# Vandermode/ELD

Hardware: AMD Instinct MI355X
Metric: raw megapixels/sec (noise-synth + U-Net step) (higher is better)
Workload: dtype f32; 1 GPU; BASELINE.json configs[1]: full ELD noise model (PGRU, SonyA7S2 params) on 4x1424x2128 packed raw + U-Net fp32 train step (fwd, L1, bwd, Adam), 8 frames per GPU; images_per_gpu=8, global_batch=8, parallelism=dp1

## Files before the change

### eld_amd/csrc/conv.h

```cpp
#pragma once
#include "common.h"

typedef float f32x16 __attribute__((ext_vector_type(16)));
typedef float f32x2 __attribute__((ext_vector_type(2)));
typedef __bf16 bf16x2_hw __attribute__((ext_vector_type(2)));

enum ConvMode { CONV_3X3 = 0, CONV_1X1 = 1, CONV_GATHER2X2 = 2 };
enum ConvEpi { EPI_FWD = 0, EPI_CONVT_FWD = 1, EPI_GRAD = 2 };

typedef unsigned short bf16_t;
enum ConvDtype { DT_F32 = 0, DT_BF16 = 1 };

struct ConvArgs {
    const void* in0;
    const void* in1;
    int C0, C1;
    const void* wp;
    int N, H, W;
    int Nout;
    int epi;
    const float* bias;
    int lrelu;
    void* out0;
    void* out1;
// ... 229 lines not shown
int launch_conv_x3w(const ConvArgs& a, hipStream_t st);
int bfd_slab_bn(int Nout, int K, int N, int H, int W);
__host__ __device__ inline size_t bfd_slab_bytes(int BN) { return (size_t)3 * BN * 64; }
int launch_conv_bfd(const ConvArgs& a, hipStream_t st);
int debug_kernel_mask(int set);
bool bfs_takes(int Nout, int K, int N, int H, int W);
int launch_conv_bfs(const ConvArgs& a, hipStream_t st);
bool bfw_takes(const ConvArgs& a);
int launch_conv_bfw(const ConvArgs& a, hipStream_t st);
int bfg_slab_bn(bool gather, int Nout, int Cs, int Cout_t, int N, int H, int W);
__host__ __device__ inline size_t bfg_slab_bytes(int BN) { return (size_t)BN * 64; }
int launch_conv_bfg(const ConvArgs& a, int mode, hipStream_t st);

#ifdef __HIPCC__
__device__ __forceinline__ int xcd_block(int on) {
    const int b = (int)blockIdx.x;
    if (!on) return b;
    const int n = (int)gridDim.x, q = n >> 3, r = n & 7, x = b & 7;
    return (x < r ? x * (q + 1) : r * (q + 1) + (x - r) * q) + (b >> 3);
}
#endif
__host__ __device__ inline void band_tile(int id, int tiles_x, int tiles_y, int BH, int& ty, int& tx) {
    if (BH <= 1) { ty = id / tiles_x; tx = id - ty * tiles_x; return; }
    const int full = tiles_x * BH, band = id / full, off = id - band * full;
    int bh = tiles_y - band * BH;
    if (bh > BH) bh = BH;
    tx = off / bh;
    ty = band * BH + (off - tx * bh);
}
int eld_tile_band();
enum { XCD_GEMM = 1, XCD_WGRAD8 = 2, XCD_WGRAD = 4, XCD_X3D = 8, XCD_X3W = 16, XCD_BF16 = 32, XCD_IGEMM = 64 };
int eld_xcd_mask();

struct WgradArgs {
    const void* g;
    int CA;
    const void* x0;
    const void* x1;
    int C0, C1;
    int N, H, W;
    float* part;
    float* bpart;
    float* xbpart;
    int CBp;
    int psplit;
    int tiles_x, tiles_y;
    int vp;
    int dtype;
    int algo;
    int wgrad8;
    int xcd;
    int band;
    const float* amax_g; const float* amax_x0; const float* amax_x1;
};

int launch_wgrad(const WgradArgs& a, int mode, hipStream_t st);
bool wgrad8_shape(int CA, int CBp, int& COB, int& JB, int& TH, int& TWo, bool bf16 = false);
int wgrad8_ntiles(int CA, int CBp, int N, int H, int W, bool bf16);
bool wgradt8_takes(int CA, int CB);
int wgradt8_ntiles(int N, int H, int W);
int launch_wgrad_reduce(const float* part, const float* bpart, float* wgrad, float* bgrad, int psplit, int T, int CA,
                        int CBp, int CBr, hipStream_t st, int bias_n = 0);
```

### eld_amd/csrc/conv_wgrad.hip

```cpp
#include <stdlib.h>
#include "conv.h"

#define TW 32
#define JB 32

typedef __bf16 bf16x8 __attribute__((ext_vector_type(8)));
typedef short s16x4 __attribute__((ext_vector_type(4)));
typedef int i32x4_t __attribute__((ext_vector_type(4)));
typedef _Float16 half8 __attribute__((ext_vector_type(8)));

enum { ALG_F32 = 0, ALG_BFM = 1, ALG_X3 = 2, ALG_H2 = 3 };

template <typename T, int MODE, int WCO, int TH, int ALG>
__global__ __launch_bounds__(256, 2) void wgrad_kernel(const WgradArgs a) {
    constexpr bool BFM = ALG == ALG_BFM, X3 = ALG == ALG_X3, H2 = ALG == ALG_H2;
    static_assert(!(X3 || H2) || sizeof(T) == 4, "x3 / h2: fp32 inputs");
    constexpr int ES = sizeof(T);
    constexpr int EPU = 16 / ES;
    constexpr int LES = X3 ? 6 : (BFM ? 2 : 4);
    constexpr int TAPS = MODE == CONV_3X3 ? 9 : 4;
    constexpr int WPIX = 4 / WCO;
    constexpr int COB = 32 * WCO;
    constexpr int TPIX = TH * TW;
    constexpr int PW = TPIX / WPIX;
// ... 320 lines not shown

    const int tid = threadIdx.x, lane = tid & 63, wave = tid >> 6;
    const int m = lane & 31, hi = lane >> 5;
    const int wco = wave % WCO, wci = (wave / WCO) % WCI, wpix = wave / (WCO * WCI);
    const int IB = a.CA / COB, JBn = a.CBp / JBK;
    int bid = xcd_block(a.xcd);
    const int jb = bid % JBn; bid /= JBn;
    const int ib = bid % IB;
    const int ps = bid / IB;
    const int i0 = ib * COB, j0 = jb * JBK;
    const bool do_bias = a.bpart != nullptr && jb == 0;

    f32x16 acc[TAPS];
#pragma unroll
    for (int t = 0; t < TAPS; ++t)
#pragma unroll
        for (int i = 0; i < 16; ++i) acc[t][i] = 0.f;
    float4 bsum4 = make_float4(0.f, 0.f, 0.f, 0.f), bsum4b = make_float4(0.f, 0.f, 0.f, 0.f);

    const int ntiles = a.tiles_x * a.tiles_y;
    const int VP = a.vp;
    const bool seam = VP % TH != 0;
    constexpr unsigned OOB = 0xFFFFFFF0u;
    constexpr int G_STEP = THREADS / G_Q;
    const int g_part = tid % G_Q, g_lp0 = tid / G_Q;
    const int g_px0 = g_lp0 % TWT, g_py0 = g_lp0 / TWT;
    const unsigned g_off0 = (unsigned)(g_px0 * a.CA + i0 + g_part * EPU) * (unsigned)ES;
    const int g_lds0 = ((g_part * EPU) >> 5) * GBLK + g_lp0 * 32 + ((g_part * EPU) & 31);
    auto g_pxy = [&](int it, int& dpx, int& dpy) {
        if (G_STEP >= TWT) { dpx = 0; dpy = it * (G_STEP / TWT); }
        else { dpx = (it * G_STEP) % TWT; dpy = (it * G_STEP) / TWT; }
    };
    const int x_part = (int)((unsigned)tid % (unsigned)XQ);
    int x_hyx[X_IT];
#pragma unroll
    for (int it = 0; it < X_IT; ++it) {
        const int hp = (int)((unsigned)(tid + it * THREADS) / (unsigned)XQ);
        const int hy = hp / (TWT + 2);
        x_hyx[it] = (hy << 8) | (hp - hy * (TWT + 2));
    }
    auto x_alive = [&](int it) { return (it + 1) * THREADS <= X_UNITS1 || (int)((unsigned)(tid + it * THREADS) / (unsigned)XQ) < X_PIX; };
    const char* xs[WCI]; int xC[WCI], xc0[WCI];
#pragma unroll
    for (int cb = 0; cb < WCI; ++cb) {
        const int c = j0 + cb * 32;
        if (c < a.C0) { xs[cb] = static_cast<const char*>(a.x0); xC[cb] = a.C0; xc0[cb] = c; }
        else if (c < a.C0 + a.C1) { xs[cb] = static_cast<const char*>(a.x1); xC[cb] = a.C1; xc0[cb] = c - a.C0; }
        else { xs[cb] = nullptr; xC[cb] = 32; xc0[cb] = 0; }
    }
    float4 rg[G_IT], rx[WCI][X_IT];
    const size_t g_img = (size_t)a.H * a.W * a.CA * ES;
    const unsigned g_rowc = (unsigned)(g_py0 * a.W * a.CA) * (unsigned)ES;
    auto load_tile = [&](int tile) {
        int ty, tx;
        band_tile(tile, a.tiles_x, a.tiles_y, a.band, ty, tx);
        const int v0 = ty * TH, x0 = tx * TWT;
        const int img0 = v0 / VP, vrel = v0 - img0 * VP;
        const int wrem = a.W - x0;
        if (!seam || VP - vrel > TH) {
            const __amdgpu_buffer_rsrc_t rs_g = __builtin_amdgcn_make_buffer_rsrc((void*)(static_cast<const char*>(a.g) + (size_t)img0 * g_img), 0, (int)g_img, 0x00020000);
            const int gbase = (vrel * a.W + x0) * a.CA * ES;
#pragma unroll
            for (int it = 0; it < G_IT; ++it) {
                int dpx, dpy;
                g_pxy(it, dpx, dpy);
                const unsigned off = g_off0 + g_rowc + (unsigned)((dpy * a.W + dpx) * a.CA) * (unsigned)ES;
                rg[it] = __builtin_bit_cast(float4, __builtin_amdgcn_raw_buffer_load_b128(rs_g, g_px0 + dpx < wrem ? (int)off : (int)OOB, gbase, 0));
            }
#pragma unroll
            for (int cb = 0; cb < WCI; ++cb) {
                const size_t x_img = (size_t)a.H * a.W * xC[cb] * ES;
                const __amdgpu_buffer_rsrc_t rs_x = __builtin_amdgcn_make_buffer_rsrc((void*)(xs[cb] ? xs[cb] + (size_t)img0 * x_img : nullptr), 0, xs[cb] ? (int)x_img : 0, 0x00020000);
#pragma unroll
                for (int it = 0; it < X_IT; ++it) {
                    const int gy = vrel - 1 + (x_hyx[it] >> 8), gx = x0 - 1 + (x_hyx[it] & 255);
                    const bool ok = x_alive(it) && (unsigned)gy < (unsigned)a.H && (unsigned)gx < (unsigned)a.W;
                    const unsigned off = ok ? (unsigned)((gy * a.W + gx) * xC[cb] + xc0[cb] + x_part * EPU) * (unsigned)ES : OOB;
                    rx[cb][it] = __builtin_bit_cast(float4, __builtin_amdgcn_raw_buffer_load_b128(rs_x, (int)off, 0, 0));
                }
            }
            return;
        }
        const int nimg = a.N - img0 < 2 ? a.N - img0 : 2;
        const int lim0 = a.H - vrel, nxt = VP - vrel;
        const __amdgpu_buffer_rsrc_t rs_g = __builtin_amdgcn_make_buffer_rsrc((void*)(static_cast<const char*>(a.g) + (size_t)img0 * g_img), 0, (int)(g_img * nimg), 0x00020000);
        const unsigned gb0 = (unsigned)((vrel * a.W + x0) * a.CA) * (unsigned)ES;
        const unsigned gb1 = (unsigned)(((a.H - nxt) * a.W + x0) * a.CA) * (unsigned)ES;
#pragma unroll
        for (int it = 0; it < G_IT; ++it) {
            int dpx, dpy;
            g_pxy(it, dpx, dpy);
            const int r = g_py0 + dpy;
            const bool second = r >= nxt;
            const bool ok = (r < lim0 || (second && r - nxt < a.H)) && g_px0 + dpx < wrem;
            const unsigned off = (second ? gb1 : gb0) + g_off0 + g_rowc + (unsigned)((dpy * a.W + dpx) * a.CA) * (unsigned)ES;
            rg[it] = __builtin_bit_cast(float4, __builtin_amdgcn_raw_buffer_load_b128(rs_g, ok ? (int)off : (int)OOB, 0, 0));
        }
#pragma unroll
        for (int cb = 0; cb < WCI; ++cb) {
            const size_t x_img = (size_t)a.H * a.W * xC[cb] * ES;
            const __amdgpu_buffer_rsrc_t rs_x = __builtin_amdgcn_make_buffer_rsrc((void*)(xs[cb] ? xs[cb] + (size_t)img0 * x_img : nullptr), 0, xs[cb] ? (int)(x_img * nimg) : 0, 0x00020000);
#pragma unroll
            for (int it = 0; it < X_IT; ++it) {
                const int r = (x_hyx[it] >> 8) - 1, gx = x0 - 1 + (x_hyx[it] & 255);
                const bool second = r >= nxt;
                const int wrow = second ? a.H + r - nxt : vrel + r;
                const bool rok = second ? r - nxt < a.H : (unsigned)(vrel + r) < (unsigned)a.H;
                const bool ok = x_alive(it) && rok && (unsigned)gx < (unsigned)a.W;
                const unsigned off = ok ? (unsigned)((wrow * a.W + gx) * xC[cb] + xc0[cb] + x_part * EPU) * (unsigned)ES : OOB;
                rx[cb][it] = __builtin_bit_cast(float4, __builtin_amdgcn_raw_buffer_load_b128(rs_x, (int)off, 0, 0));
            }
        }
    };
    auto put3 = [&](bf16_t* d, int plane_elems, const float4& raw) {
        if constexpr (ES == 2) { *reinterpret_cast<float4*>(d) = raw; return; }
        const unsigned x0 = __float_as_uint(raw.x), x1 = __float_as_uint(raw.y), x2 = __float_as_uint(raw.z), x3 = __float_as_uint(raw.w);
        const float r0 = raw.x - __uint_as_float(x0 & 0xFFFF0000u), r1 = raw.y - __uint_as_float(x1 & 0xFFFF0000u);
        const float r2 = raw.z - __uint_as_float(x2 & 0xFFFF0000u), r3 = raw.w - __uint_as_float(x3 & 0xFFFF0000u);
        const unsigned y0 = __float_as_uint(r0), y1 = __float_as_uint(r1), y2 = __float_as_uint(r2), y3 = __float_as_uint(r3);
        const unsigned z0 = __float_as_uint(r0 - __uint_as_float(y0 & 0xFFFF0000u)), z1 = __float_as_uint(r1 - __uint_as_float(y1 & 0xFFFF0000u));
        const unsigned z2 = __float_as_uint(r2 - __uint_as_float(y2 & 0xFFFF0000u)), z3 = __float_as_uint(r3 - __uint_as_float(y3 & 0xFFFF0000u));
        auto hp = [](unsigned lo, unsigned hi_) { return __builtin_amdgcn_perm(hi_, lo, 0x07060302u); };
        *reinterpret_cast<uint2*>(d) = make_uint2(hp(x0, x1), hp(x2, x3));
        *reinterpret_cast<uint2*>(d + plane_elems) = make_uint2(hp(y0, y1), hp(y2, y3));
        *reinterpret_cast<uint2*>(d + 2 * plane_elems) = make_uint2(hp(z0, z1), hp(z2, z3));
    };
    auto store_tile = [&]() {
#pragma unroll
        for (int it = 0; it < G_IT; ++it) {
            put3(ldsG + g_lds0 + it * G_STEP * 32, GPL, rg[it]);
            if (do_bias) {
                if constexpr (ES == 4) { bsum4.x += rg[it].x; bsum4.y += rg[it].y; bsum4.z += rg[it].z; bsum4.w += rg[it].w; }
                else {
                    const uint4 q = __builtin_bit_cast(uint4, rg[it]);
                    const float4 lo = unpack_bf4(make_uint2(q.x, q.y)), hi4 = unpack_bf4(make_uint2(q.z, q.w));
                    bsum4.x += lo.x; bsum4.y += lo.y; bsum4.z += lo.z; bsum4.w += lo.w;
                    bsum4b.x += hi4.x; bsum4b.y += hi4.y; bsum4b.z += hi4.z; bsum4b.w += hi4.w;
                }
            }
        }
#pragma unroll
        for (int cb = 0; cb < WCI; ++cb)
#pragma unroll
            for (int it = 0; it < X_IT; ++it)
                if (x_alive(it)) put3(ldsX + (cb * X_PIX + (int)((unsigned)(tid + it * THREADS) / (unsigned)XQ)) * 32 + x_part * EPU, XPL, rx[cb][it]);
    };

    const int gi = lane & 15, gg = lane >> 4;
    constexpr bool ROWSHARE = STREAM == 2;
    static_assert(!ROWSHARE || (NPC == 3 && TWT == 8 && WPIX == 1 && TH % 2 == 0), "row-shared fragments: fp32, 8-pixel-wide tiles, one pixel slice");
    constexpr int HS = TH / 2;
    const int lq0 = ROWSHARE ? HS * TWT * hi + (gi >> 2) : wpix * PW + 8 * hi + (gi >> 2);
    const int pyq = lq0 / TWT, pxq = lq0 - pyq * TWT;
    const bf16_t* gq = ldsG + wco * GBLK + lq0 * 32 + (gg & 1) * 16 + (gi & 3) * 4;
    const bf16_t* xq = ldsX + (wci * X_PIX + pyq * (TWT + 2) + pxq) * 32 + (gg & 1) * 16 + (gi & 3) * 4;
    auto tr8 = [](const bf16_t* p0) {
        const s16x4 lo = __builtin_amdgcn_ds_read_tr16_b64_v4i16((__attribute__((address_space(3))) s16x4*)p0);
        const s16x4 hi4 = __builtin_amdgcn_ds_read_tr16_b64_v4i16((__attribute__((address_space(3))) s16x4*)(p0 + 4 * 32));
        return __builtin_bit_cast(bf16x8, __builtin_shufflevector(lo, hi4, 0, 1, 2, 3, 4, 5, 6, 7));
    };

    if (ps < ntiles) load_tile(ps);
    for (int tile = ps; tile < ntiles; tile += a.psplit) {
        __syncthreads();
        store_tile();
        __syncthreads();
        if (tile + a.psplit < ntiles) load_tile(tile + a.psplit);
        if constexpr (ROWSHARE) {
            constexpr int GI[6] = {0, 1, 2, 0, 1, 0};
            constexpr int XI[6] = {2, 1, 0, 1, 0, 0};
            constexpr int NU = (HS + 2) * 3;
            bf16x8 gr[3][3], xf[2][3];
            auto readG = [&](int s_, bf16x8 (&g3)[3]) {
#pragma unroll
                for (int pc = 0; pc < 3; ++pc) g3[pc] = tr8(gq + pc * GPL + s_ * TWT * 32);
            };
            auto readF = [&](int a_, int kx, bf16x8 (&x3)[3]) {
#pragma unroll
                for (int pc = 0; pc < 3; ++pc) x3[pc] = tr8(xq + pc * XPL + (a_ * (TWT + 2) + kx) * 32);
            };
            readG(0, gr[0]);
            readF(0, 0, xf[0]);
#pragma unroll
            for (int u = 0; u < NU; ++u) {
                const int a_ = u / 3, kx = u % 3;
                if (u + 1 < NU) readF((u + 1) / 3, (u + 1) % 3, xf[(u + 1) & 1]);
                __builtin_amdgcn_sched_barrier(0);
#pragma unroll
                for (int ky = 2; ky >= 0; --ky) {
                    const int s_ = a_ - ky;
                    if (s_ >= 0 && s_ < HS) {
#pragma unroll
                        for (int q = 0; q < 6; ++q)
                            acc[3 * ky + kx] = __builtin_amdgcn_mfma_f32_32x32x16_bf16(gr[s_ % 3][GI[q]], xf[u & 1][XI[q]], acc[3 * ky + kx], 0, 0, 0);
                    }
                    if (ky == 2 && kx == 2 && a_ + 1 < HS) {
                        __builtin_amdgcn_sched_barrier(0);
                        readG(a_ + 1, gr[(a_ + 1) % 3]);
                    }
                }
                __builtin_amdgcn_sched_barrier(0);
            }
        } else
        if constexpr (NPC == 3 && STREAM == 1) {
            constexpr int GI[6] = {0, 1, 2, 0, 1, 0};
            constexpr int XI[6] = {2, 1, 0, 1, 0, 0};
            constexpr int NBLK = KSB * TAPS;
            bf16x8 ga[2][3], xb[2][3];
            auto readG = [&](int ks, bf16x8 (&g3)[3]) {
#pragma unroll
                for (int pc = 0; pc < 3; ++pc) g3[pc] = tr8(gq + pc * GPL + ks * 16 * 32);
            };
            auto readX = [&](int ks, int t, bf16x8 (&x3)[3]) {
                const int lrel = ks * 16, dy0 = lrel / TWT, dxp = lrel - dy0 * TWT;
                const int xoff = (dy0 + t / 3) * (TWT + 2) + dxp + t % 3;
#pragma unroll
                for (int pc = 0; pc < 3; ++pc) x3[pc] = tr8(xq + pc * XPL + xoff * 32);
            };
            readG(0, ga[0]);
            readX(0, 0, xb[0]);
// ... 25 lines not shown
                for (int tt = 0; tt < 3; ++tt) {
                    const int xoff = (dy0 + t0 / 3) * (TWT + 2) + dxp + tt;
#pragma unroll
                    for (int pc = 0; pc < NPC; ++pc) xb[tt][pc] = tr8(xq + pc * XPL + xoff * 32);
                }
                if constexpr (NPC == 3) {
                    constexpr int GI[6] = {0, 1, 2, 0, 1, 0};
                    constexpr int XI[6] = {2, 1, 0, 1, 0, 0};
#pragma unroll
                    for (int q = 0; q < 6; ++q)
#pragma unroll
                        for (int tt = 0; tt < 3; ++tt)
                            acc[t0 + tt] = __builtin_amdgcn_mfma_f32_32x32x16_bf16(ga[GI[q]], xb[tt][XI[q]], acc[t0 + tt], 0, 0, 0);
                } else {
#pragma unroll
                    for (int tt = 0; tt < 3; ++tt) acc[t0 + tt] = __builtin_amdgcn_mfma_f32_32x32x16_bf16(ga[0], xb[tt][0], acc[t0 + tt], 0, 0, 0);
                }
                __builtin_amdgcn_sched_barrier(0);
            }
        }
    }

    __syncthreads();
    float* red = lds;
    const size_t pbase = (size_t)ps * TAPS * a.CA * a.CBp;
    const int wt = wci * WCO + wco;
#pragma unroll
    for (int t = 0; t < TAPS; ++t) {
        if (WPIX > 1) {
            if (wpix > 0) {
#pragma unroll
                for (int i = 0; i < 16; ++i) red[(((wpix - 1) * (WCO * WCI) + wt) * 16 + i) * 64 + lane] = acc[t][i];
            }
            __syncthreads();
            if (wpix == 0) {
                for (int w = 0; w < WPIX - 1; ++w)
#pragma unroll
                    for (int i = 0; i < 16; ++i) acc[t][i] += red[((w * (WCO * WCI) + wt) * 16 + i) * 64 + lane];
            }
            __syncthreads();
        }
        if (wpix == 0) {
#pragma unroll
            for (int i = 0; i < 16; ++i) {
                const int row = (i & 3) + 8 * (i >> 2) + 4 * hi;
                a.part[pbase + ((size_t)t * a.CA + i0 + wco * 32 + row) * a.CBp + j0 + wci * 32 + m] = acc[t][i];
            }
        }
    }
    if (do_bias) {
        __syncthreads();
        if constexpr (ES == 4) reinterpret_cast<float4*>(red)[tid] = bsum4;
        else { reinterpret_cast<float4*>(red)[2 * tid] = bsum4; reinterpret_cast<float4*>(red)[2 * tid + 1] = bsum4b; }
        __syncthreads();
        if (tid < COB) {
            const int q = tid / EPU, comp = tid % EPU;
            float s_ = 0.f;
            for (int k = 0; k < THREADS / G_Q; ++k) s_ += red[(q + k * G_Q) * EPU + comp];
            a.bpart[(size_t)ps * a.CA + i0 + tid] = s_;
        }
    }
}

__device__ __forceinline__ void wg_dma16(i32x4_t rsrc, unsigned voff, unsigned lds_dst) {
    unsigned keep;
    asm volatile("s_nop 4\n\ts_mov_b32 %0, m0\n\ts_mov_b32 m0, %3\n\ts_nop 0\n\tbuffer_load_dwordx4 %1, %2, 0 offen lds\n\ts_mov_b32 m0, %0"
                 : "=&s"(keep) : "v"(voff), "s"(rsrc), "s"(lds_dst) : "memory");
}

template <int WCO, int WCI, int WPIX, int TH, int TWT>
__global__ __launch_bounds__(512, 2) void wgrad8d_kernel(const WgradArgs a) {
    static_assert(WCO * WCI * WPIX == 8, "8 waves");
    static_assert(TWT == 8 || TWT == 16 || TWT == 32, "tile width");
    constexpr int WAVES = 8, THREADS = 512, TAPS = 9;
    constexpr int COB = 32 * WCO, JBK = 32 * WCI, TPIX = TH * TWT, PW = TPIX / WPIX, KSB = PW / 16;
    static_assert(PW % 16 == 0 && PW >= 16, "a wave's pixel slice is a whole number of 16-pixel k-steps");
    constexpr int HW = TWT + 2, X_PIX = (TH + 2) * HW;
    static_assert((TPIX * 4) % 64 == 0, "a block of G is whole DMA pieces");
    constexpr int GB_PIECES = TPIX * 4 / 64, XB_PIECES = (X_PIX * 4 + 63) / 64;
    constexpr int G_PIECES = WCO * GB_PIECES, X_PIECES = WCI * XB_PIECES;
    constexpr int G_IT = (G_PIECES + WAVES - 1) / WAVES, X_IT = (X_PIECES + WAVES - 1) / WAVES;
    constexpr int GBLK = GB_PIECES * 512, XBLK = XB_PIECES * 512;
    constexpr int BUF_BYTES = (G_PIECES + X_PIECES) * 1024;
    extern __shared__ __attribute__((aligned(16))) float lds[];

    const int tid = threadIdx.x, lane = tid & 63;
    const int wave = __builtin_amdgcn_readfirstlane(tid >> 6);
    const int m = lane & 31, hi = lane >> 5;
    const int wco = wave % WCO, wci = (wave / WCO) % WCI, wpix = wave / (WCO * WCI);
    const int IB = a.CA / COB, JBn = a.CBp / JBK;
    int bid = xcd_block(a.xcd);
    const int jb = bid % JBn; bid /= JBn;
    const int ib = bid % IB;
    const int ps = bid / IB;
    const int i0 = ib * COB, j0 = jb * JBK;
    const bool do_bias = a.bpart != nullptr && jb == 0;

    f32x16 acc[TAPS];
#pragma unroll
    for (int t = 0; t < TAPS; ++t)
#pragma unroll
        for (int i = 0; i < 16; ++i) acc[t][i] = 0.f;
    float4 bsum4 = make_float4(0.f, 0.f, 0.f, 0.f), bsum4b = make_float4(0.f, 0.f, 0.f, 0.f);

    const int ntiles = a.tiles_x * a.tiles_y;
    const int VP = a.vp;
// ... 313 lines not shown
            const int cb = tid >> 5, c = tid & 31, quad = c >> 2, comp = c & 3;
            float s_ = 0.f;
            for (int k = 0; k < THREADS / 8; ++k) s_ += reinterpret_cast<const float*>(&r[cb * THREADS + quad + 8 * k])[comp];
            a.xbpart[(size_t)ps * a.CBp + j0 + tid] = s_;
        }
    }
}

bool wgradt8_takes(int CA, int CB) {
    static const int on = [] { const char* e = getenv("ELD_WGRADT8"); return e ? atoi(e) : 1; }();
    return on && CA % 128 == 0 && CB % 64 == 0;
}
int wgradt8_ntiles(int N, int H, int W) { return ((W + 7) / 8) * ((H + 7) / 8) * N; }

static int launch_wt8(WgradArgs a, hipStream_t st) {
    eld_note_conv_kernel("wgradt8");
    a.xcd = eld_xcd_mask() & XCD_WGRAD8;
    a.band = eld_tile_band();
    a.tiles_x = (a.W + 7) / 8;
    a.tiles_y = (a.H + 7) / 8;
    const size_t lds_bytes = (size_t)(3 * 4 * (64 * 32 + 32) + 3 * 2 * 256 * 32) * 2;
    const long long blocks = (long long)(a.CA / 128) * (a.CBp / 64) * a.psplit;
    if (blocks <= 0) return 0;
    if ((size_t)4 * a.H * a.W * a.C0 * 4 >= 0xFFFFFFF0ull || (size_t)a.H * a.W * a.CA * 4 >= 0xFFFFFFF0ull) return ELD_ENOTSUP;
    auto kern = wgradt8_kernel<0>;
    static EldAttrOnce once;
    { const int rc = once.ensure(kern, lds_bytes); if (rc) return rc; }
    ELD_LAUNCH(kern, dim3((unsigned)blocks), dim3(512), lds_bytes, st, a);
    ELD_LAUNCH_CHECK();
    return 0;
}

bool wgrad8_shape(int CA, int CBp, int& COB, int& JBK, int& TH, int& TWo, bool bf16) {
    if (CA % 32 || CBp % 32) return false;
    TWo = 32;
    if (CA % 128 == 0 && CBp % 64 == 0) { COB = 128; JBK = 64; TH = 2; }
    else if (CA % 64 == 0 && CBp % 64 == 0) { COB = 64; JBK = 64; TH = 2; }
    else if (CA % 64 == 0) { COB = 64; JBK = 32; TH = 4; }
    else if (CBp % 64 == 0) { COB = 32; JBK = 64; TH = 4; }
    else { COB = 32; JBK = 32; TH = 4; }
    if (bf16) TH = 8;
    if (bf16 && wgrad8_dma() && COB == 128) { TH = 16; TWo = 8; return true; }
    if (COB == 128) { TH = TH * 4; TWo = 8; }
    return true;
}

int wgrad8_ntiles(int CA, int CBp, int N, int H, int W, bool bf16) {
    int COB, JBK, TH, TWo;
    if (!wgrad8_shape(CA, CBp, COB, JBK, TH, TWo, bf16)) return 0;
    const int VP = vrow_pitch(N, H, TH);
    return ((W + TWo - 1) / TWo) * ((vrow_extent(N, H, VP) + TH - 1) / TH);
}

template <typename T, int WCO, int WCI, int WPIX, int TH, int TWT, int STREAM = 0>
static int launch_w8(WgradArgs a, hipStream_t st) {
    eld_note_conv_kernel(sizeof(T) == 2 ? "wgrad8<bf16>" : "wgrad8<f32>");
    a.xcd = eld_xcd_mask() & XCD_WGRAD8;
    a.band = eld_tile_band();
    constexpr int COB = 32 * WCO, JBK = 32 * WCI;
    a.vp = vrow_pitch(a.N, a.H, TH);
    a.tiles_x = (a.W + TWT - 1) / TWT;
    a.tiles_y = (vrow_extent(a.N, a.H, a.vp) + TH - 1) / TH;
    size_t lds_bytes = (size_t)((TH * TWT * 32 + (sizeof(T) == 4 ? 32 : 0)) * (COB / 32) + (TH + 2) * (TWT + 2) * JBK) * (sizeof(T) == 4 ? 6 : 2);
    const size_t red_bytes = (size_t)7 * 16 * 64 * sizeof(float) * 1;
    if (lds_bytes < red_bytes) lds_bytes = red_bytes;
    const long long blocks = (long long)(a.CA / COB) * (a.CBp / JBK) * a.psplit;
    if (blocks <= 0) return 0;
    auto kern = wgrad8_kernel<T, WCO, WCI, WPIX, TH, TWT, STREAM>;
    static EldAttrOnce once;
    { const int rc = once.ensure(kern, lds_bytes); if (rc) return rc; }
    ELD_LAUNCH(kern, dim3((unsigned)blocks), dim3(512), lds_bytes, st, a);
    ELD_LAUNCH_CHECK();
    return 0;
}

template <int WCO, int WCI, int WPIX, int TH, int TWT>
static int launch_w8d(WgradArgs a, hipStream_t st) {
    eld_note_conv_kernel("wgrad8d");
    a.xcd = eld_xcd_mask() & XCD_WGRAD8;
    a.band = eld_tile_band();
    constexpr int COB = 32 * WCO, JBK = 32 * WCI;
    a.vp = vrow_pitch(a.N, a.H, TH);
    a.tiles_x = (a.W + TWT - 1) / TWT;
    a.tiles_y = (vrow_extent(a.N, a.H, a.vp) + TH - 1) / TH;
    constexpr int PIECES = WCO * (TH * TWT * 4 / 64) + WCI * (((TH + 2) * (TWT + 2) * 4 + 63) / 64);
    size_t lds_bytes = (size_t)2 * PIECES * 1024;
    const size_t red_bytes = (size_t)7 * 16 * 64 * sizeof(float);
    if (lds_bytes < red_bytes) lds_bytes = red_bytes;
    const long long blocks = (long long)(a.CA / COB) * (a.CBp / JBK) * a.psplit;
    if (blocks <= 0) return 0;
    auto kern = wgrad8d_kernel<WCO, WCI, WPIX, TH, TWT>;
    static EldAttrOnce once;
    { const int rc = once.ensure(kern, lds_bytes); if (rc) return rc; }
    ELD_LAUNCH(kern, dim3((unsigned)blocks), dim3(512), lds_bytes, st, a);
    ELD_LAUNCH_CHECK();
    return 0;
}

static int launch_wgrad8(const WgradArgs& a, hipStream_t st) {
    const bool bf16 = a.dtype == DT_BF16;
    const size_t es = bf16 ? 2 : 4;
    int COB, JBK, TH, TWo;
    if (!wgrad8_shape(a.CA, a.CBp, COB, JBK, TH, TWo, bf16)) return ELD_ENOTSUP;
    if ((a.C0 % 32) || (a.C1 % 32)) return ELD_ENOTSUP;
    const size_t win = a.N > 1 ? 2 : 1;
    if ((size_t)a.H * a.W * a.CA * es * win >= 0xFFFFFFF0ull || (size_t)a.H * a.W * (a.C0 > a.C1 ? a.C0 : a.C1) * es * win >= 0xFFFFFFF0ull) return ELD_ENOTSUP;
    if (bf16 && wgrad8_dma() && COB == 128) {
        return launch_w8d<4, 2, 1, 16, 8>(a, st);
    }
    if (bf16) {
        if (COB == 128) return launch_w8<bf16_t, 4, 2, 1, 32, 8>(a, st);
        if (COB == 64 && JBK == 64) return launch_w8<bf16_t, 2, 2, 2, 8, 32>(a, st);
        if (COB == 64) return launch_w8<bf16_t, 2, 1, 4, 8, 32>(a, st);
        if (JBK == 64) return launch_w8<bf16_t, 1, 2, 4, 8, 32>(a, st);
        return launch_w8<bf16_t, 1, 1, 8, 8, 32>(a, st);
    }
    static const int stream = [] { const char* e = getenv("ELD_WG8_STREAM"); return e ? atoi(e) : 0; }();
    static const int rowshare = [] { const char* e = getenv("ELD_WG8_ROWSHARE"); return e ? atoi(e) : 0; }();
    if (COB == 128 && rowshare) return launch_w8<float, 4, 2, 1, 8, 8, 2>(a, st);
    if (COB == 128) return (stream & 1) ? launch_w8<float, 4, 2, 1, 8, 8, 1>(a, st) : launch_w8<float, 4, 2, 1, 8, 8>(a, st);
    if (stream & 2) {
        if (COB == 64 && JBK == 64) return launch_w8<float, 2, 2, 2, 2, 32, 1>(a, st);
        if (COB == 64) return launch_w8<float, 2, 1, 4, 4, 32, 1>(a, st);
        if (JBK == 64) return launch_w8<float, 1, 2, 4, 4, 32, 1>(a, st);
        return launch_w8<float, 1, 1, 8, 4, 32, 1>(a, st);
    }
    if (COB == 64 && JBK == 64) return launch_w8<float, 2, 2, 2, 2, 32>(a, st);
    if (COB == 64) return launch_w8<float, 2, 1, 4, 4, 32>(a, st);
    if (JBK == 64) return launch_w8<float, 1, 2, 4, 4, 32>(a, st);
    return launch_w8<float, 1, 1, 8, 4, 32>(a, st);
}

template <typename T, int MODE, int WCO, int TH, int ALG = ALG_F32>
static int launch_w(WgradArgs a, hipStream_t st) {
    eld_note_conv_kernel(sizeof(T) == 2 ? (MODE == CONV_3X3 ? "wgrad<bf16>" : "wgrad<bf16,gather>") : (MODE == CONV_3X3 ? "wgrad<f32>" : "wgrad<f32,gather>"));
    a.xcd = eld_xcd_mask() & XCD_WGRAD;
    constexpr int COB = 32 * WCO;
    constexpr int X_PIX = MODE == CONV_3X3 ? (TH + 2) * (TW + 2) : 4 * TH * TW;
    a.tiles_x = (a.W + TW - 1) / TW;
    a.tiles_y = (a.H + TH - 1) / TH;
    constexpr int GROWS = TH * TW + ((ALG == ALG_X3 || ALG == ALG_H2) ? 1 : 0);
    size_t lds_bytes = (size_t)(GROWS * COB + X_PIX * JB) * (ALG == ALG_X3 ? 6 : (ALG == ALG_BFM ? 2 : 4));
    const size_t red_bytes = (size_t)4 * 16 * 64 * sizeof(float);
    if (lds_bytes < red_bytes) lds_bytes = red_bytes;
    const long long blocks = (long long)(a.CA / COB) * (a.CBp / JB) * a.psplit;
    if (blocks <= 0) return 0;
    auto kern = wgrad_kernel<T, MODE, WCO, TH, ALG>;
    static EldAttrOnce once;
    { const int rc = once.ensure(kern, lds_bytes); if (rc) return rc; }
    ELD_LAUNCH(kern, dim3((unsigned)blocks), dim3(256), lds_bytes, st, a);
    ELD_LAUNCH_CHECK();
    return 0;
}

int launch_wgrad(const WgradArgs& a, int mode, hipStream_t st) {
    if (a.CA % 32 || a.CBp % 32 || a.C0 % 4 || a.C1 % 4 || a.psplit < 1) return ELD_EINVAL;
    if (a.C1 > 0 && a.C0 % 32) return ELD_EINVAL;
    const bool c64 = a.CA % 64 == 0;
    if (a.dtype == DT_BF16) {
        if (a.C0 % 8 || a.C1 % 8) return ELD_EINVAL;
        if (mode == CONV_3X3 && a.wgrad8) {
            const int rc = launch_wgrad8(a, st);
            if (rc != ELD_ENOTSUP) return rc;
        }
        static const int mma = [] { const char* e = getenv("ELD_WGRAD_BF16_MMA"); return e ? atoi(e) : 1; }();
        if (mma) {
            if (mode == CONV_3X3) return c64 ? launch_w<bf16_t, CONV_3X3, 2, 4, ALG_BFM>(a, st) : launch_w<bf16_t, CONV_3X3, 1, 4, ALG_BFM>(a, st);
            if (mode == CONV_GATHER2X2) return c64 ? launch_w<bf16_t, CONV_GATHER2X2, 2, 2, ALG_BFM>(a, st) : launch_w<bf16_t, CONV_GATHER2X2, 1, 2, ALG_BFM>(a, st);
            return ELD_EINVAL;
        }
        if (mode == CONV_3X3) return c64 ? launch_w<bf16_t, CONV_3X3, 2, 4>(a, st) : launch_w<bf16_t, CONV_3X3, 1, 4>(a, st);
        if (mode == CONV_GATHER2X2) return c64 ? launch_w<bf16_t, CONV_GATHER2X2, 2, 2>(a, st) : launch_w<bf16_t, CONV_GATHER2X2, 1, 2>(a, st);
        return ELD_EINVAL;
    }
    const int algo = resolve_algo(a.algo);
    if (algo == 2) {
        if (!a.amax_g || !a.amax_x0) return ELD_EINVAL;
        if (mode == CONV_3X3) return c64 ? launch_w<float, CONV_3X3, 2, 2, ALG_H2>(a, st) : launch_w<float, CONV_3X3, 1, 4, ALG_H2>(a, st);
        if (mode == CONV_GATHER2X2) return c64 ? launch_w<float, CONV_GATHER2X2, 2, 2, ALG_H2>(a, st) : launch_w<float, CONV_GATHER2X2, 1, 2, ALG_H2>(a, st);
// ... 93 lines not shown
```

Baseline: 727.1 raw MPix/s.

## Add double-buffered warp-specialized fp32 wgrad8 kernel for small channel blocks

Adds a new wgrad8w kernel that keeps two LDS tile buffers, so staging the next tile (split into three bf16 planes) overlaps with the MFMA work on the current one. Half the waves stage before their MFMAs and half after, to spread LDS and VMEM traffic, and only one barrier is needed per tile. It is enabled by default for fp32 blocks with 64x64 and 32x32 channels. It also adds debug-flag early exits gated by a dev-tools env var. The cost is twice the LDS footprint, which may reduce occupancy.

```diff
diff --git a/eld_amd/csrc/conv.h b/eld_amd/csrc/conv.h
--- a/eld_amd/csrc/conv.h
+++ b/eld_amd/csrc/conv.h
@@ -305,6 +305,7 @@
     int xcd;
     int band;
     const float* amax_g; const float* amax_x0; const float* amax_x1;
+    int dbg;
 };
 
 int launch_wgrad(const WgradArgs& a, int mode, hipStream_t st);
diff --git a/eld_amd/csrc/conv_wgrad.hip b/eld_amd/csrc/conv_wgrad.hip
--- a/eld_amd/csrc/conv_wgrad.hip
+++ b/eld_amd/csrc/conv_wgrad.hip
@@ -396,6 +396,7 @@
     const size_t g_img = (size_t)a.H * a.W * a.CA * ES;
     const unsigned g_rowc = (unsigned)(g_py0 * a.W * a.CA) * (unsigned)ES;
     auto load_tile = [&](int tile) {
+        if (ELD_DBG(a) & 4) return;
         int ty, tx;
         band_tile(tile, a.tiles_x, a.tiles_y, a.band, ty, tx);
         const int v0 = ty * TH, x0 = tx * TWT;
@@ -470,6 +471,7 @@
         *reinterpret_cast<uint2*>(d + 2 * plane_elems) = make_uint2(hp(z0, z1), hp(z2, z3));
     };
     auto store_tile = [&]() {
+        if (ELD_DBG(a) & 16) return;
 #pragma unroll
         for (int it = 0; it < G_IT; ++it) {
             put3(ldsG + g_lds0 + it * G_STEP * 32, GPL, rg[it]);
@@ -510,6 +512,7 @@
         store_tile();
         __syncthreads();
         if (tile + a.psplit < ntiles) load_tile(tile + a.psplit);
+        if (ELD_DBG(a) & 2) continue;
         if constexpr (ROWSHARE) {
             constexpr int GI[6] = {0, 1, 2, 0, 1, 0};
             constexpr int XI[6] = {2, 1, 0, 1, 0, 0};
@@ -641,6 +644,268 @@
         __syncthreads();
         if constexpr (ES == 4) reinterpret_cast<float4*>(red)[tid] = bsum4;
         else { reinterpret_cast<float4*>(red)[2 * tid] = bsum4; reinterpret_cast<float4*>(red)[2 * tid + 1] = bsum4b; }
+        __syncthreads();
+        if (tid < COB) {
+            const int q = tid / EPU, comp = tid % EPU;
+            float s_ = 0.f;
+            for (int k = 0; k < THREADS / G_Q; ++k) s_ += red[(q + k * G_Q) * EPU + comp];
+            a.bpart[(size_t)ps * a.CA + i0 + tid] = s_;
+        }
+    }
+}
+
+template <int WCO, int WCI, int WPIX, int TH, int TWT>
+__global__ __launch_bounds__(512, 2) void wgrad8w_kernel(const WgradArgs a) {
+    constexpr int ES = 4, EPU = 4, NPC = 3, XQ = 8;
+    static_assert(WCO * WCI * WPIX == 8, "8 waves");
+    constexpr int THREADS = 512, TAPS = 9;
+    constexpr int COB = 32 * WCO, JBK = 32 * WCI, TPIX = TH * TWT, PW = TPIX / WPIX, KSB = PW / 16;
+    static_assert(TWT == 8 || TWT == 16 || TWT == 32, "tile width");
+    static_assert(PW % 16 == 0 && PW >= 16, "a wave's pixel slice is a whole number of 16-pixel k-steps");
+    constexpr int X_PIX = (TH + 2) * (TWT + 2);
+    constexpr int GBLK = TPIX * 32 + 32;
+    constexpr int GPL = GBLK * WCO, XPL = X_PIX * JBK;
+    constexpr int G_Q = COB / EPU, G_UNITS = TPIX * G_Q, G_IT = G_UNITS / THREADS;
+    static_assert(G_UNITS % THREADS == 0 && THREADS % G_Q == 0, "a thread stages the same channel quad of G in every iteration");
+    constexpr int X_UNITS1 = X_PIX * XQ, X_IT = (X_UNITS1 + THREADS - 1) / THREADS;
+    constexpr int BUFE = NPC * (GPL + XPL);
+    static_assert(2 * BUFE * 2 <= 160 * 1024, "two tile buffers must fit the LDS");
+    extern __shared__ __attribute__((aligned(16))) float lds[];
+    bf16_t* ldsG = reinterpret_cast<bf16_t*>(lds);
+    bf16_t* ldsX = ldsG + NPC * GPL;
+
+    const int tid = threadIdx.x, lane = tid & 63, wave = tid >> 6;
+    const int m = lane & 31, hi = lane >> 5;
+    const int wco = wave % WCO, wci = (wave / WCO) % WCI, wpix = wave / (WCO * WCI);
+    const int IB = a.CA / COB, JBn = a.CBp / JBK;
+    int bid = xcd_block(a.xcd);
+    const int jb = bid % JBn; bid /= JBn;
+    const int ib = bid % IB;
+    const int ps = bid / IB;
+    const int i0 = ib * COB, j0 = jb * JBK;
+    const bool do_bias = a.bpart != nullptr && jb == 0;
+
+    f32x16 acc[TAPS];
+#pragma unroll
+    for (int t = 0; t < TAPS; ++t)
+#pragma unroll
+        for (int i = 0; i < 16; ++i) acc[t][i] = 0.f;
+    float4 bsum4 = make_float4(0.f, 0.f, 0.f, 0.f);
+
+    const int ntiles = a.tiles_x * a.tiles_y;
+    const int VP = a.vp;
+    const bool seam = VP % TH != 0;
+    constexpr unsigned OOB = 0xFFFFFFF0u;
+    constexpr int G_STEP = THREADS / G_Q;
+    const int g_part = tid % G_Q, g_lp0 = tid / G_Q;
+    const int g_px0 = g_lp0 % TWT, g_py0 = g_lp0 / TWT;
+    const unsigned g_off0 = (unsigned)(g_px0 * a.CA + i0 + g_part * EPU) * (unsigned)ES;
+    const int g_lds0 = ((g_part * EPU) >> 5) * GBLK + g_lp0 * 32 + ((g_part * EPU) & 31);
+    auto g_pxy = [&](int it, int& dpx, int& dpy) {
+        if (G_STEP >= TWT) { dpx = 0; dpy = it * (G_STEP / TWT); }
+        else { dpx = (it * G_STEP) % TWT; dpy = (it * G_STEP) / TWT; }
+    };
+    const int x_part = (int)((unsigned)tid % (unsigned)XQ);
+    int x_hyx[X_IT];
+#pragma unroll
+    for (int it = 0; it < X_IT; ++it) {
+        const int hp = (int)((unsigned)(tid + it * THREADS) / (unsigned)XQ);
+        const int hy = hp / (TWT + 2);
+        x_hyx[it] = (hy << 8) | (hp - hy * (TWT + 2));
+    }
+    auto x_alive = [&](int it) { return (it + 1) * THREADS <= X_UNITS1 || (int)((unsigned)(tid + it * THREADS) / (unsigned)XQ) < X_PIX; };
+    const char* xs[WCI]; int xC[WCI], xc0[WCI];
+#pragma unroll
+    for (int cb = 0; cb < WCI; ++cb) {
+        const int c = j0 + cb * 32;
+        if (c < a.C0) { xs[cb] = static_cast<const char*>(a.x0); xC[cb] = a.C0; xc0[cb] = c; }
+        else if (c < a.C0 + a.C1) { xs[cb] = static_cast<const char*>(a.x1); xC[cb] = a.C1; xc0[cb] = c - a.C0; }
+        else { xs[cb] = nullptr; xC[cb] = 32; xc0[cb] = 0; }
+    }
+    float4 rg[G_IT], rx[WCI][X_IT];
+    const size_t g_img = (size_t)a.H * a.W * a.CA * ES;
+    const unsigned g_rowc = (unsigned)(g_py0 * a.W * a.CA) * (unsigned)ES;
+    auto load_tile = [&](int tile) {
+        if (ELD_DBG(a) & 4) return;
+        int ty, tx;
+        band_tile(tile, a.tiles_x, a.tiles_y, a.band, ty, tx);
+        const int v0 = ty * TH, x0 = tx * TWT;
+        const int img0 = v0 / VP, vrel = v0 - img0 * VP;
+        const int wrem = a.W - x0;
+        if (!seam || VP - vrel > TH) {
+            const __amdgpu_buffer_rsrc_t rs_g = __builtin_amdgcn_make_buffer_rsrc((void*)(static_cast<const char*>(a.g) + (size_t)img0 * g_img), 0, (int)g_img, 0x00020000);
+            const int gbase = (vrel * a.W + x0) * a.CA * ES;
+#pragma unroll
+            for (int it = 0; it < G_IT; ++it) {
+                int dpx, dpy;
+                g_pxy(it, dpx, dpy);
+                const unsigned off = g_off0 + g_rowc + (unsigned)((dpy * a.W + dpx) * a.CA) * (unsigned)ES;
+                rg[it] = __builtin_bit_cast(float4, __builtin_amdgcn_raw_buffer_load_b128(rs_g, g_px0 + dpx < wrem ? (int)off : (int)OOB, gbase, 0));
+            }
+#pragma unroll
+            for (int cb = 0; cb < WCI; ++cb) {
+                const size_t x_img = (size_t)a.H * a.W * xC[cb] * ES;
+                const __amdgpu_buffer_rsrc_t rs_x = __builtin_amdgcn_make_buffer_rsrc((void*)(xs[cb] ? xs[cb] + (size_t)img0 * x_img : nullptr), 0, xs[cb] ? (int)x_img : 0, 0x00020000);
+#pragma unroll
+                for (int it = 0; it < X_IT; ++it) {
+                    const int gy = vrel - 1 + (x_hyx[it] >> 8), gx = x0 - 1 + (x_hyx[it] & 255);
+                    const bool ok = x_alive(it) && (unsigned)gy < (unsigned)a.H && (unsigned)gx < (unsigned)a.W;
+                    const unsigned off = ok ? (unsigned)((gy * a.W + gx) * xC[cb] + xc0[cb] + x_part * EPU) * (unsigned)ES : OOB;
+                    rx[cb][it] = __builtin_bit_cast(float4, __builtin_amdgcn_raw_buffer_load_b128(rs_x, (int)off, 0, 0));
+                }
+            }
+            return;
+        }
+        const int nimg = a.N - img0 < 2 ? a.N - img0 : 2;
+        const int lim0 = a.H - vrel, nxt = VP - vrel;
+        const __amdgpu_buffer_rsrc_t rs_g = __builtin_amdgcn_make_buffer_rsrc((void*)(static_cast<const char*>(a.g) + (size_t)img0 * g_img), 0, (int)(g_img * nimg), 0x00020000);
+        const unsigned gb0 = (unsigned)((vrel * a.W + x0) * a.CA) * (unsigned)ES;
+        const unsigned gb1 = (unsigned)(((a.H - nxt) * a.W + x0) * a.CA) * (unsigned)ES;
+#pragma unroll
+        for (int it = 0; it < G_IT; ++it) {
+            int dpx, dpy;
+            g_pxy(it, dpx, dpy);
+            const int r = g_py0 + dpy;
+            const bool second = r >= nxt;
+            const bool ok = (r < lim0 || (second && r - nxt < a.H)) && g_px0 + dpx < wrem;
+            const unsigned off = (second ? gb1 : gb0) + g_off0 + g_rowc + (unsigned)((dpy * a.W + dpx) * a.CA) * (unsigned)ES;
+            rg[it] = __builtin_bit_cast(float4, __builtin_amdgcn_raw_buffer_load_b128(rs_g, ok ? (int)off : (int)OOB, 0, 0));
+        }
+#pragma unroll
+        for (int cb = 0; cb < WCI; ++cb) {
+            const size_t x_img = (size_t)a.H * a.W * xC[cb] * ES;
+            const __amdgpu_buffer_rsrc_t rs_x = __builtin_amdgcn_make_buffer_rsrc((void*)(xs[cb] ? xs[cb] + (size_t)img0 * x_img : nullptr), 0, xs[cb] ? (int)(x_img * nimg) : 0, 0x00020000);
+#pragma unroll
+            for (int it = 0; it < X_IT; ++it) {
+                const int r = (x_hyx[it] >> 8) - 1, gx = x0 - 1 + (x_hyx[it] & 255);
+                const bool second = r >= nxt;
+                const int wrow = second ? a.H + r - nxt : vrel + r;
+                const bool rok = second ? r - nxt < a.H : (unsigned)(vrel + r) < (unsigned)a.H;
+                const bool ok = x_alive(it) && rok && (unsigned)gx < (unsigned)a.W;
+                const unsigned off = ok ? (unsigned)((wrow * a.W + gx) * xC[cb] + xc0[cb] + x_part * EPU) * (unsigned)ES : OOB;
+                rx[cb][it] = __builtin_bit_cast(float4, __builtin_amdgcn_raw_buffer_load_b128(rs_x, (int)off, 0, 0));
+            }
+        }
+    };
+    auto put3 = [&](bf16_t* d, int plane_elems, const float4& raw) {
+        const unsigned x0 = __float_as_uint(raw.x), x1 = __float_as_uint(raw.y), x2 = __float_as_uint(raw.z), x3 = __float_as_uint(raw.w);
+        const float r0 = raw.x - __uint_as_float(x0 & 0xFFFF0000u), r1 = raw.y - __uint_as_float(x1 & 0xFFFF0000u);
+        const float r2 = raw.z - __uint_as_float(x2 & 0xFFFF0000u), r3 = raw.w - __uint_as_float(x3 & 0xFFFF0000u);
+        const unsigned y0 = __float_as_uint(r0), y1 = __float_as_uint(r1), y2 = __float_as_uint(r2), y3 = __float_as_uint(r3);
+        const unsigned z0 = __float_as_uint(r0 - __uint_as_float(y0 & 0xFFFF0000u)), z1 = __float_as_uint(r1 - __uint_as_float(y1 & 0xFFFF0000u));
+        const unsigned z2 = __float_as_uint(r2 - __uint_as_float(y2 & 0xFFFF0000u)), z3 = __float_as_uint(r3 - __uint_as_float(y3 & 0xFFFF0000u));
+        auto hp = [](unsigned lo, unsigned hi_) { return __builtin_amdgcn_perm(hi_, lo, 0x07060302u); };
+        *reinterpret_cast<uint2*>(d) = make_uint2(hp(x0, x1), hp(x2, x3));
+        *reinterpret_cast<uint2*>(d + plane_elems) = make_uint2(hp(y0, y1), hp(y2, y3));
+        *reinterpret_cast<uint2*>(d + 2 * plane_elems) = make_uint2(hp(z0, z1), hp(z2, z3));
+    };
+    auto store_tile = [&](int bo) {
+        if (ELD_DBG(a) & 16) return;
+#pragma unroll
+        for (int it = 0; it < G_IT; ++it) {
+            put3(ldsG + bo + g_lds0 + it * G_STEP * 32, GPL, rg[it]);
+            if (do_bias) { bsum4.x += rg[it].x; bsum4.y += rg[it].y; bsum4.z += rg[it].z; bsum4.w += rg[it].w; }
+        }
+#pragma unroll
+        for (int cb = 0; cb < WCI; ++cb)
+#pragma unroll
+            for (int it = 0; it < X_IT; ++it)
+                if (x_alive(it)) put3(ldsX + bo + (cb * X_PIX + (int)((unsigned)(tid + it * THREADS) / (unsigned)XQ)) * 32 + x_part * EPU, XPL, rx[cb][it]);
+    };
+
+    const int gi = lane & 15, gg = lane >> 4;
+    const int lq0 = wpix * PW + 8 * hi + (gi >> 2);
+    const int pyq = lq0 / TWT, pxq = lq0 - pyq * TWT;
+    const bf16_t* gq0 = ldsG + wco * GBLK + lq0 * 32 + (gg & 1) * 16 + (gi & 3) * 4;
+    const bf16_t* xq0 = ldsX + (wci * X_PIX + pyq * (TWT + 2) + pxq) * 32 + (gg & 1) * 16 + (gi & 3) * 4;
+    auto tr8 = [](const bf16_t* p0) {
+        const s16x4 lo = __builtin_amdgcn_ds_read_tr16_b64_v4i16((__attribute__((address_space(3))) s16x4*)p0);
+        const s16x4 hi4 = __builtin_amdgcn_ds_read_tr16_b64_v4i16((__attribute__((address_space(3))) s16x4*)(p0 + 4 * 32));
+        return __builtin_bit_cast(bf16x8, __builtin_shufflevector(lo, hi4, 0, 1, 2, 3, 4, 5, 6, 7));
+    };
+
+    auto mma_tile = [&](const bf16_t* gq, const bf16_t* xq) {
+        if (ELD_DBG(a) & 2) return;
+#pragma unroll
+        for (int ks = 0; ks < KSB; ++ks) {
+            const int lrel = ks * 16;
+            const int dy0 = lrel / TWT, dxp = lrel - dy0 * TWT;
+            bf16x8 ga[NPC];
+#pragma unroll
+            for (int pc = 0; pc < NPC; ++pc) ga[pc] = tr8(gq + pc * GPL + lrel * 32);
+#pragma unroll
+            for (int t0 = 0; t0 < TAPS; t0 += 3) {
+                bf16x8 xb[3][NPC];
+#pragma unroll
+                for (int tt = 0; tt < 3; ++tt) {
+                    const int xoff = (dy0 + t0 / 3) * (TWT + 2) + dxp + tt;
+#pragma unroll
+                    for (int pc = 0; pc < NPC; ++pc) xb[tt][pc] = tr8(xq + pc * XPL + xoff * 32);
+                }
+                constexpr int GI[6] = {0, 1, 2, 0, 1, 0};
+                constexpr int XI[6] = {2, 1, 0, 1, 0, 0};
+#pragma unroll
+                for (int q = 0; q < 6; ++q)
+#pragma unroll
+                    for (int tt = 0; tt < 3; ++tt)
+                        acc[t0 + tt] = __builtin_amdgcn_mfma_f32_32x32x16_bf16(ga[GI[q]], xb[tt][XI[q]], acc[t0 + tt], 0, 0, 0);
+                __builtin_amdgcn_sched_barrier(0);
+            }
+        }
+    };
+
+    const bool late = (__builtin_amdgcn_readfirstlane(tid >> 6) & 4) != 0;
+    const int step = a.psplit;
+    if (ps < ntiles) {
+        load_tile(ps);
+        store_tile(0);
+        if (ps + step < ntiles) load_tile(ps + step);
+    }
+    __syncthreads();
+    int bo = 0;
+    for (int tile = ps; tile < ntiles; tile += step) {
+        const bool more = tile + step < ntiles;
+        auto stage_next = [&]() {
+            store_tile(bo ^ BUFE);
+            if (tile + 2 * step < ntiles) load_tile(tile + 2 * step);
+        };
+        if (late && more) stage_next();
+        mma_tile(gq0 + bo, xq0 + bo);
+        if (!late && more) stage_next();
+        __syncthreads();
+        bo ^= BUFE;
+    }
+
+    __syncthreads();
+    float* red = lds;
+    const size_t pbase = (size_t)ps * TAPS * a.CA * a.CBp;
+    const int wt = wci * WCO + wco;
+#pragma unroll
+    for (int t = 0; t < TAPS; ++t) {
+        if (WPIX > 1) {
+            if (wpix > 0) {
+#pragma unroll
+                for (int i = 0; i < 16; ++i) red[(((wpix - 1) * (WCO * WCI) + wt) * 16 + i) * 64 + lane] = acc[t][i];
+            }
+            __syncthreads();
+            if (wpix == 0) {
+                for (int w = 0; w < WPIX - 1; ++w)
+#pragma unroll
+                    for (int i = 0; i < 16; ++i) acc[t][i] += red[((w * (WCO * WCI) + wt) * 16 + i) * 64 + lane];
+            }
+            __syncthreads();
+        }
+        if (wpix == 0) {
+#pragma unroll
+            for (int i = 0; i < 16; ++i) {
+                const int row = (i & 3) + 8 * (i >> 2) + 4 * hi;
+                a.part[pbase + ((size_t)t * a.CA + i0 + wco * 32 + row) * a.CBp + j0 + wci * 32 + m] = acc[t][i];
+            }
+        }
+    }
+    if (do_bias) {
+        __syncthreads();
+        reinterpret_cast<float4*>(red)[tid] = bsum4;
         __syncthreads();
         if (tid < COB) {
             const int q = tid / EPU, comp = tid % EPU;
@@ -1060,11 +1325,19 @@
     return ((W + TWo - 1) / TWo) * ((vrow_extent(N, H, VP) + TH - 1) / TH);
 }
 
+static void wgrad8_dbg(WgradArgs& a) {
+    a.dbg = 0;
+#if ELD_DEV_TOOLS
+    { static const int dbg = [] { const char* e = getenv("ELD_CONV_DBG"); return e ? atoi(e) : 0; }(); a.dbg = dbg; }
+#endif
+}
+
 template <typename T, int WCO, int WCI, int WPIX, int TH, int TWT, int STREAM = 0>
 static int launch_w8(WgradArgs a, hipStream_t st) {
     eld_note_conv_kernel(sizeof(T) == 2 ? "wgrad8<bf16>" : "wgrad8<f32>");
     a.xcd = eld_xcd_mask() & XCD_WGRAD8;
     a.band = eld_tile_band();
+    wgrad8_dbg(a);
     constexpr int COB = 32 * WCO, JBK = 32 * WCI;
     a.vp = vrow_pitch(a.N, a.H, TH);
     a.tiles_x = (a.W + TWT - 1) / TWT;
@@ -1075,6 +1348,27 @@
     const long long blocks = (long long)(a.CA / COB) * (a.CBp / JBK) * a.psplit;
     if (blocks <= 0) return 0;
     auto kern = wgrad8_kernel<T, WCO, WCI, WPIX, TH, TWT, STREAM>;
+    static EldAttrOnce once;
+    { const int rc = once.ensure(kern, lds_bytes); if (rc) return rc; }
+    ELD_LAUNCH(kern, dim3((unsigned)blocks), dim3(512), lds_bytes, st, a);
+    ELD_LAUNCH_CHECK();
+    return 0;
+}
+
+template <int WCO, int WCI, int WPIX, int TH, int TWT>
+static int launch_w8w(WgradArgs a, hipStream_t st) {
+    eld_note_conv_kernel("wgrad8w<f32>");
+    a.xcd = eld_xcd_mask() & XCD_WGRAD8;
+    a.band = eld_tile_band();
+    wgrad8_dbg(a);
+    constexpr int COB = 32 * WCO, JBK = 32 * WCI;
+    a.vp = vrow_pitch(a.N, a.H, TH);
+    a.tiles_x = (a.W + TWT - 1) / TWT;
+    a.tiles_y = (vrow_extent(a.N, a.H, a.vp) + TH - 1) / TH;
+    const size_t lds_bytes = (size_t)2 * ((TH * TWT * 32 + 32) * (COB / 32) + (TH + 2) * (TWT + 2) * JBK) * 6;
+    const long long blocks = (long long)(a.CA / COB) * (a.CBp / JBK) * a.psplit;
+    if (blocks <= 0) return 0;
+    auto kern = wgrad8w_kernel<WCO, WCI, WPIX, TH, TWT>;
     static EldAttrOnce once;
     { const int rc = once.ensure(kern, lds_bytes); if (rc) return rc; }
     ELD_LAUNCH(kern, dim3((unsigned)blocks), dim3(512), lds_bytes, st, a);
@@ -1133,6 +1427,9 @@
         if (JBK == 64) return launch_w8<float, 1, 2, 4, 4, 32, 1>(a, st);
         return launch_w8<float, 1, 1, 8, 4, 32, 1>(a, st);
     }
+    static const int wg8w = [] { const char* e = getenv("ELD_WG8W"); return e ? atoi(e) : 1; }();
+    if (wg8w && COB == 64 && JBK == 64) return launch_w8w<2, 2, 2, 2, 32>(a, st);
+    if (wg8w && COB == 32 && JBK == 32) return launch_w8w<1, 1, 8, 4, 32>(a, st);
     if (COB == 64 && JBK == 64) return launch_w8<float, 2, 2, 2, 2, 32>(a, st);
     if (COB == 64) return launch_w8<float, 2, 1, 4, 4, 32>(a, st);
     if (JBK == 64) return launch_w8<float, 1, 2, 4, 4, 32>(a, st);
```

Measured after the change: 732.4 raw MPix/s, median of 6. Within noise of the previous version (+0.7%).
